# gau-nernst/llama-x

Measured on AMD Instinct MI355X. Metric: train tokens/sec Llama-3.1-8B seq4096 at 1/2/4/8 MI355X; p50 step ms, higher is better.
Workload: dtype bf16; 1 GPU; Llama-3.1-8B text-only LoRA r=16 bf16, seq=4096, 1 sequence per GPU, causal mask, base+LM head frozen (BASELINE.json configs[1]); random-init weights at 8B dimensions; seq_len=4096, parallelism=dp1, launch=hipGraph replay (fwd+bwd+AdamW), lm_head_rows=labelled only

## Files before the change

### llama-x_amd/csrc/attn_bwd.hip

```cpp
#include "attn.h"
#include "attn_dropout.h"

typedef __attribute__((ext_vector_type(8))) short s16x8_t;

__device__ __forceinline__ int dual_swz(int row) { return ((row & 3) << 2) | ((row >> 2) & 3); }
__device__ __forceinline__ uint32_t dual_swz(uint32_t row) { return ((row & 3) << 2) | ((row >> 2) & 3); }

__device__ __forceinline__ bf16x8_t tr_frag(const char* img, int row0, int db, int lane) {
  const int hh = lane >> 5, tq = (lane & 15) >> 2, tp = lane & 3, tsub = (lane >> 4) & 1;
  const int chunk = 4 * db + 2 * tsub + (tp >> 1);
  const int rlo = row0 + 4 * hh + tq, rhi = rlo + 8;
  s16x4_t lo = __builtin_amdgcn_ds_read_tr16_b64_v4i16((lds_s16x4*)(img + rlo * 256 + ((chunk ^ dual_swz(rlo)) << 4) + ((tp & 1) << 3)));
  s16x4_t hi = __builtin_amdgcn_ds_read_tr16_b64_v4i16((lds_s16x4*)(img + rhi * 256 + ((chunk ^ dual_swz(rhi)) << 4) + ((tp & 1) << 3)));
  s16x8_t v = {lo[0], lo[1], lo[2], lo[3], hi[0], hi[1], hi[2], hi[3]};
  return __builtin_bit_cast(bf16x8_t, v);
}

__device__ __forceinline__ bf16x8_t row_frag(const char* img, int row, int ks, int hh) {
  return *reinterpret_cast<const bf16x8_t*>(img + row * 256 + (((2 * ks + hh) ^ dual_swz(row)) << 4));
}

template <int N>
__device__ __forceinline__ void lds_tr_wait(s16x4_t& a, s16x4_t& b, s16x4_t (&c)[4], s16x4_t (&d)[4]) {
  asm volatile("s_waitcnt lgkmcnt(%10)"
               : "+v"(a), "+v"(b), "+v"(c[0]), "+v"(c[1]), "+v"(c[2]), "+v"(c[3]), "+v"(d[0]), "+v"(d[1]), "+v"(d[2]), "+v"(d[3])
               : "n"(N));
  __builtin_amdgcn_sched_barrier(0);
}
__device__ __forceinline__ uint32_t xor_imm(uint32_t a, int c) {
  if (c == 0) return a;
  uint32_t r;
  asm volatile("v_xor_b32 %0, %1, %2" : "=v"(r) : "n"(c), "v"(a));
  return r;
}

struct AttnBwdArgs {
  const bf16_t* q; const bf16_t* k; const bf16_t* v; const bf16_t* o; const bf16_t* d_o;
  const float* lse; float* delta; float* nlse;
  const float* rope;
  unsigned long long* stamps;
  bf16_t* dq; bf16_t* dk; bf16_t* dv;
  bf16_t* ds; int Sp;
  int64_t q_sb, q_ss, k_sb, k_ss, v_sb, v_ss, o_sb, o_ss, do_sb, do_ss;
  int64_t dq_sb, dq_ss, dk_sb, dk_ss, dv_sb, dv_ss;
  const int* doc_ids; const int* prefix_len; const uint8_t* flags;
  int B, S, H, KVH;
  float scale, scale_log2;
  const uint8_t* mask; int64_t m_sb, m_sq;
  const int64_t* rng; uint32_t drop_thr; float drop_c; int stream_id;
};

enum { BWD_CAUSAL = 0, BWD_RULE = 1, BWD_MASK = 2 };

__device__ __forceinline__ uint32_t mask_nibble(uint32_t w) {
  const uint32_t nz = (((w & 0x7f7f7f7fu) + 0x7f7f7f7fu) | w) & 0x80808080u;
  return ((nz >> 7) * 0x01020408u) >> 24;
}

#define DQ_STAGE_BYTES (2 * TILE_BYTES)
#define DQ_LDS_BYTES (2 * DQ_STAGE_BYTES)

template <int MODE, bool DROPOUT = false>
__global__ __launch_bounds__(256, 2) void attn_bwd_dq_kernel(const AttnBwdArgs a) {
  static_assert(!(DROPOUT && MODE == BWD_MASK), "dropout exists in the causal and the rule mode");
  constexpr bool GENERAL = MODE == BWD_RULE;
  constexpr bool FLAGS = MODE != BWD_CAUSAL;
  constexpr bool MASK = MODE == BWD_MASK;
  extern __shared__ __attribute__((aligned(256))) char smem[];
  const int tid = threadIdx.x, lane = tid & 63;
  const int wave = __builtin_amdgcn_readfirstlane(tid >> 6);
  const int nqb = (a.S + BQ - 1) / BQ, nkt = (a.S + BKV - 1) / BKV;
  const int qb = nqb - 1 - blockIdx.y;
  const int h = blockIdx.x, b = blockIdx.z;
  const int kvh = h / (a.H / a.KVH);
  const int r = lane & 31, hh = lane >> 5;
  const int qi = qb * BQ + wave * 32 + r;
  const int qrow = min(qi, a.S - 1);

  const uint8_t* fl = FLAGS ? a.flags + ((int64_t)b * nqb + qb) * nkt : nullptr;
  const int kt_end = FLAGS ? nkt : min(nkt, (qb * BQ + BQ + BKV - 1) / BKV);
  uint32_t fpack = 0;
  int fchunk = -1;
  auto tile_class = [&](int t) -> int {
    if constexpr (FLAGS) {
      if ((t >> 6) != fchunk) {
        fchunk = t >> 6;
        fpack = fl[min(fchunk * 64 + lane, nkt - 1)];
      }
      return __builtin_amdgcn_readlane((int)fpack, t & 63);
    } else {
      return (t * BKV + BKV - 1 <= qb * BQ) ? 2 : 1;
    }
  };
  auto next_tile = [&](int t) {
    while (t < kt_end && tile_class(t) == 0) ++t;
    return t;
  };

  const int srow_in = lane >> 4, sslot = lane & 15;
  const bf16_t* kbase = a.k + (int64_t)b * a.k_sb + kvh * HD;
  const bf16_t* vbase = a.v + (int64_t)b * a.v_sb + kvh * HD;
  uint32_t koff[4], voff[4];
#pragma unroll
  for (int i = 0; i < 4; ++i) {
    const int row = i * 16 + wave * 4 + srow_in;
    koff[i] = (uint32_t)(((int64_t)row * a.k_ss + (sslot ^ dual_swz(row)) * 8) * 2);
    voff[i] = (uint32_t)(((int64_t)row * a.v_ss + (sslot ^ (row & 15)) * 8) * 2);
  }
  auto stage = [&](int buf, int t) {
    char* sK = smem + buf * DQ_STAGE_BYTES;
    char* sV = sK + TILE_BYTES;
    if (t * BKV + BKV <= a.S) {
      const char* kt = (const char*)(kbase + (int64_t)t * BKV * a.k_ss);
      const char* vt = (const char*)(vbase + (int64_t)t * BKV * a.v_ss);
      if constexpr (DROPOUT) {
        uint32_t l0;
        asm volatile("v_mbcnt_lo_u32_b32 %0, -1, 0\n\tv_mbcnt_hi_u32_b32 %0, -1, %0" : "=v"(l0));
        const int slot = (int)(l0 & 15);
#pragma unroll
        for (int i = 0; i < 4; ++i) {
          const int row = i * 16 + wave * 4 + (int)(l0 >> 4);
          const uint32_t ko = (uint32_t)(((int64_t)row * a.k_ss + (slot ^ dual_swz(row)) * 8) * 2);
          const uint32_t vo = (uint32_t)(((int64_t)row * a.v_ss + (slot ^ (row & 15)) * 8) * 2);
          __builtin_amdgcn_global_load_lds((gbl_void*)(kt + ko), (lds_void*)(sK + (i * 16 + wave * 4) * 256), 16, 0, 0);
          __builtin_amdgcn_global_load_lds((gbl_void*)(vt + vo), (lds_void*)(sV + (i * 16 + wave * 4) * 256), 16, 0, 0);
        }
      } else {
#pragma unroll
      for (int i = 0; i < 4; ++i) {
        __builtin_amdgcn_global_load_lds((gbl_void*)(kt + koff[i]), (lds_void*)(sK + (i * 16 + wave * 4) * 256), 16, 0, 0);
        __builtin_amdgcn_global_load_lds((gbl_void*)(vt + voff[i]), (lds_void*)(sV + (i * 16 + wave * 4) * 256), 16, 0, 0);
      }
      }
    } else {
#pragma unroll
      for (int i = 0; i < 4; ++i) {
        const int row = i * 16 + wave * 4 + srow_in;
        const int key = min(t * BKV + row, a.S - 1);
        const int kc = sslot ^ dual_swz(row);
        const int vc = sslot ^ (row & 15);
        __builtin_amdgcn_global_load_lds((gbl_void*)(kbase + (int64_t)key * a.k_ss + kc * 8), (lds_void*)(sK + (i * 16 + wave * 4) * 256), 16, 0, 0);
        __builtin_amdgcn_global_load_lds((gbl_void*)(vbase + (int64_t)key * a.v_ss + vc * 8), (lds_void*)(sV + (i * 16 + wave * 4) * 256), 16, 0, 0);
      }
    }
  };

  const uint32_t sbase = (uint32_t)(uintptr_t)(__attribute__((address_space(3))) char*)smem;
  uint32_t aK0;
  {
    const int tq2 = (lane & 15) >> 2, tp = lane & 3, tsub = (lane >> 4) & 1;
    const int rlo = 4 * hh + tq2;
    aK0 = (uint32_t)(rlo * 256 + (((2 * tsub + (tp >> 1)) ^ dual_swz(rlo)) << 4) + ((tp & 1) << 3));
  }
  f32x16_t dq[4];
#pragma unroll
  for (int i = 0; i < 4; ++i)
#pragma unroll
    for (int e = 0; e < 16; ++e) dq[i][e] = 0.f;
  const int* docrow = (GENERAL && a.doc_ids) ? a.doc_ids + (int64_t)b * a.S : nullptr;
  const int my_doc = docrow ? docrow[qrow] : 0;
  const int my_prefix = (GENERAL && a.prefix_len) ? a.prefix_len[b] : 0;
  uint32_t mwn[MASK ? 8 : 1];
  auto mask_request = [&](int t_) {
    if constexpr (MASK) {
      uint32_t l0;
      asm volatile("v_mbcnt_lo_u32_b32 %0, -1, 0\n\tv_mbcnt_hi_u32_b32 %0, -1, %0" : "=v"(l0));
      const int hh = (int)(l0 >> 5);
      const uint8_t* mrow = a.mask + (int64_t)b * a.m_sb + (int64_t)min(qb * BQ + wave * 32 + (int)(l0 & 31), a.S - 1) * a.m_sq;
      if (t_ * BKV + BKV <= a.S) {
        const uint8_t* p = mrow + t_ * BKV + 4 * hh;
#pragma unroll
        for (int g = 0; g < 8; ++g) __builtin_memcpy(&mwn[g], p + (g >> 2) * 32 + 8 * (g & 3), 4);
      } else {
#pragma unroll
        for (int g = 0; g < 8; ++g) {
          const int g0 = t_ * BKV + (g >> 2) * 32 + 8 * (g & 3) + 4 * hh;
          __builtin_memcpy(&mwn[g], mrow + min(g0, a.S - 4), 4);
        }
      }
    }
  };
  auto mask_bits = [&](int t_) -> uint32_t {
    uint32_t bits = 0;
    if constexpr (MASK) {
      const bool ragged = t_ * BKV + BKV > a.S;
#pragma unroll
      for (int g = 0; g < 8; ++g) {
        uint32_t w = mwn[g];
        if (ragged) {
          const int g0 = t_ * BKV + (g >> 2) * 32 + 8 * (g & 3) + 4 * hh;
          const int sh = g0 - min(g0, a.S - 4);
          w = sh >= 4 ? 0u : w >> (8 * sh);
        }
        bits |= mask_nibble(w) << (4 * g);
      }
    }
    return bits;
  };

  int t = next_tile(0);
  if constexpr (MASK) {
#pragma unroll
    for (int g = 0; g < 8; ++g) mwn[g] = 0;
    if (t < kt_end && tile_class(t) == 1) mask_request(t);
  }
  if (t < kt_end) stage(0, t);
  bf16x8_t qf[8], dof[8], ovf[8];
  const float my_lse = a.lse[((int64_t)b * a.H + h) * a.S + qrow];
  {
    const bf16_t* qp = a.q + (int64_t)b * a.q_sb + (int64_t)qrow * a.q_ss + h * HD + 8 * hh;
    const bf16_t* dp = a.d_o + (int64_t)b * a.do_sb + (int64_t)qrow * a.do_ss + h * HD + 8 * hh;
    const bf16_t* op = a.o + (int64_t)b * a.o_sb + (int64_t)qrow * a.o_ss + h * HD + 8 * hh;
#pragma unroll
    for (int ks = 0; ks < 8; ++ks) {
      ovf[ks] = *reinterpret_cast<const bf16x8_t*>(op + 16 * ks);
      dof[ks] = *reinterpret_cast<const bf16x8_t*>(dp + 16 * ks);
      qf[ks] = *reinterpret_cast<const bf16x8_t*>(qp + 16 * ks);
    }
    __builtin_amdgcn_sched_barrier(0);
  }
  const float lse_safe = (my_lse == -INFINITY) ? 0.f : my_lse;
  float my_delta = 0.f;
  {
#pragma unroll
    for (int ks = 0; ks < 8; ++ks) {
#pragma unroll
      for (int j = 0; j < 8; ++j) my_delta += (float)ovf[ks][j] * (float)dof[ks][j];
    }
    my_delta += __shfl_xor(my_delta, 32, 64);
    if (hh == 0 && qi < a.S) {
      a.delta[((int64_t)b * a.H + h) * a.S + qi] = my_delta;
      a.nlse[((int64_t)b * a.H + h) * a.S + qi] = -lse_safe;
    }
  }

  asm volatile("s_waitcnt vmcnt(0)" ::: "memory");
  __syncthreads();
  int cur = 0;
  int docv = (GENERAL && docrow && t < kt_end) ? docrow[min(t * BKV + lane, a.S - 1)] : 0, docv_next = 0;
  AttnDropKey dkey = {0u, 0u};
  if constexpr (DROPOUT) dkey = attn_dropout_key(a.rng[0], a.rng[1], a.stream_id, b, h);
  while (t < kt_end) {
    int cls_m = 0;
    uint32_t mbits = 0;
    if constexpr (MASK) {
      cls_m = tile_class(t);
      if (cls_m == 1) mbits = mask_bits(t);
    }
    const int tn = next_tile(t + 1);
    if (tn < kt_end) stage(cur ^ 1, tn);
    if (GENERAL && docrow && tn < kt_end) docv_next = docrow[min(tn * BKV + lane, a.S - 1)];
    if constexpr (MASK) {
      if (tn < kt_end && tile_class(tn) == 1) mask_request(tn);
    }
    const char* sK = smem + cur * DQ_STAGE_BYTES;
    const char* sV = sK + TILE_BYTES;
    const int cls = MASK ? cls_m : tile_class(t);
#pragma unroll
    for (int kb = 0; kb < 2; ++kb) {
      f32x16_t st, dp;
      const f32x16_t zero = {0.f, 0.f, 0.f, 0.f, 0.f, 0.f, 0.f, 0.f, 0.f, 0.f, 0.f, 0.f, 0.f, 0.f, 0.f, 0.f};
      const int row = kb * 32 + r;
#pragma unroll
      for (int ks = 0; ks < 8; ++ks) {
        bf16x8_t kf = row_frag(sK, row, ks, hh);
        st = __builtin_amdgcn_mfma_f32_32x32x16_bf16(kf, qf[ks], ks == 0 ? zero : st, 0, 0, 0);
      }
      if (cls != 2) {
#pragma unroll
        for (int e = 0; e < 16; ++e) {
          if constexpr (MASK) {
            st[e] = ((mbits >> (kb * 16 + e)) & 1u) ? st[e] : -INFINITY;
          } else {
          const int kk = t * BKV + kb * 32 + (e & 3) + 8 * (e >> 2) + 4 * hh;
          bool ok = (kk < a.S) && (kk <= qi || kk < my_prefix);
          if constexpr (GENERAL) {
            const int kd = docrow ? __builtin_amdgcn_ds_bpermute((kk - t * BKV) << 2, docv) : my_doc;
            ok = ok && (kd == my_doc);
          }
          st[e] = ok ? st[e] : -INFINITY;
          }
        }
      }
#pragma unroll
      for (int e = 0; e < 16; ++e) st[e] = __builtin_amdgcn_exp2f(__builtin_fmaf(st[e], a.scale_log2, -lse_safe));
#pragma unroll
      for (int ks = 0; ks < 8; ++ks) {
        bf16x8_t vf = *reinterpret_cast<const bf16x8_t*>(sV + row * 256 + (((2 * ks + hh) ^ (row & 15)) << 4));
        dp = __builtin_amdgcn_mfma_f32_32x32x16_bf16(vf, dof[ks], ks == 0 ? zero : dp, 0, 0, 0);
      }
#pragma unroll
      for (int e = 0; e < 16; ++e) {
        float dpe = dp[e];
        if constexpr (DROPOUT) {
          const int kk = t * BKV + kb * 32 + (e & 3) + 8 * (e >> 2) + 4 * hh;
          dpe = attn_drop_keep(attn_drop_row(dkey, qi), attn_drop_col(dkey, kk), a.drop_thr) ? dpe * a.drop_c : 0.f;
        }
        st[e] = st[e] * (dpe - my_delta);
      }
      {
        const uint32_t kb_ = sbase + cur * DQ_STAGE_BYTES + kb * 8192 + aK0;
        s16x4_t Kl[4], Kh[4];
#pragma unroll
        for (int s = 0; s < 2; ++s) {
#pragma unroll
          for (int db = 0; db < 4; ++db) {
            if (s == 0) { lds_tr_read<0>(Kl[db], xor_imm(kb_, db << 6)); lds_tr_read<2048>(Kh[db], xor_imm(kb_, (db << 6) | 0x20)); }
            else { lds_tr_read<4096>(Kl[db], xor_imm(kb_, db << 6)); lds_tr_read<4096 + 2048>(Kh[db], xor_imm(kb_, (db << 6) | 0x20)); }
          }
          bf16x8_t dsb;
#pragma unroll
          for (int j = 0; j < 8; ++j) dsb[j] = (__bf16)st[8 * s + j];
          lds_tr_wait8<0>(Kl, Kh);
#pragma unroll
          for (int db = 0; db < 4; ++db) dq[db] = __builtin_amdgcn_mfma_f32_32x32x16_bf16(frag_of(Kl[db], Kh[db]), dsb, dq[db], 0, 0, 0);
          __builtin_amdgcn_sched_barrier(0);
        }
      }
    }
    asm volatile("s_waitcnt vmcnt(0)" ::: "memory");
    __syncthreads();
    cur ^= 1;
    t = tn;
    docv = docv_next;
  }

  if (qi < a.S) {
    bf16_t* op = a.dq + (int64_t)b * a.dq_sb + (int64_t)qi * a.dq_ss + h * HD;
    const bool wide = ((((uintptr_t)a.dq) | (uintptr_t)(a.dq_ss * 2) | (uintptr_t)(a.dq_sb * 2)) & 15) == 0;
#pragma unroll
    for (int db = 0; db < 4; ++db)
#pragma unroll
      for (int j2 = 0; j2 < 2; ++j2) {
        u32x2_t pp[2];
#pragma unroll
        for (int gg = 0; gg < 2; ++gg) {
          const int g4 = 2 * j2 + gg;
          u32x2_t pk;
          pk[0] = pack_bf2(dq[db][4 * g4 + 0] * a.scale, dq[db][4 * g4 + 1] * a.scale);
          pk[1] = pack_bf2(dq[db][4 * g4 + 2] * a.scale, dq[db][4 * g4 + 3] * a.scale);
          if (a.rope) {
            const f32x4_t t = *reinterpret_cast<const f32x4_t*>(a.rope + ((int64_t)qi * 64 + ((32 * db + 8 * g4 + 4 * hh) >> 1)) * 2);
            const float c0 = t[0], s0 = t[1] * -1.f, c1 = t[2], s1 = t[3] * -1.f;
            const float x0 = bflo(pk[0]), x1 = bfhi(pk[0]), y0 = bflo(pk[1]), y1 = bfhi(pk[1]);
            pk[0] = pack_bf2(x0 * c0 - x1 * s0, x1 * c0 + x0 * s0);
            pk[1] = pack_bf2(y0 * c1 - y1 * s1, y1 * c1 + y0 * s1);
          }
          pp[gg] = pk;
        }
        if (wide) {
          const auto r0 = __builtin_amdgcn_permlane32_swap(pp[0][0], pp[1][0], false, false);
          const auto r1 = __builtin_amdgcn_permlane32_swap(pp[0][1], pp[1][1], false, false);
          *reinterpret_cast<u32x4_t*>(op + 32 * db + 16 * j2 + 8 * hh) = u32x4_t{r0[0], r1[0], r0[1], r1[1]};
        } else {
          *reinterpret_cast<u32x2_t*>(op + 32 * db + 16 * j2 + 4 * hh) = pp[0];
          *reinterpret_cast<u32x2_t*>(op + 32 * db + 16 * j2 + 8 + 4 * hh) = pp[1];
        }
      }
  }
}

#define DKV_QT 64
#define DKV2_KEYS 128

typedef __attribute__((address_space(3))) char lds_char;
typedef __attribute__((address_space(3))) bf16x8_t lds_bf16x8;
typedef __attribute__((address_space(3))) f32x4_t lds_f32x4;
#define DKV3_LDS_BYTES (0x10000 + 1024)

template <int MODE, bool STAMP = false, bool DS = false, bool DROPOUT = false>
__global__ __launch_bounds__(256, 2) void attn_bwd_dkv3_kernel(const AttnBwdArgs a, float* __restrict__ part) {
  static_assert(!(DROPOUT && (MODE == BWD_MASK || STAMP || DS)), "dropout exists on the default route, in the causal and the rule mode");
  constexpr bool GENERAL = MODE == BWD_RULE;
  constexpr bool FLAGS = MODE != BWD_CAUSAL;
  constexpr bool MASK = MODE == BWD_MASK;
  static_assert(!(MASK && (STAMP || DS)), "the dense-mask mode exists on the default route only");
  extern __shared__ __attribute__((aligned(256))) char smem[];
  const int tid = threadIdx.x, lane = tid & 63;
  const int wave = __builtin_amdgcn_readfirstlane(tid >> 6);
  const int nqb = (a.S + BQ - 1) / BQ, nkt = (a.S + BKV - 1) / BKV;
  const int nqt = (a.S + DKV_QT - 1) / DKV_QT;
  const int G = a.H / a.KVH;
  int id = blockIdx.x;
  const int per_kb = a.B * a.KVH * G;
  const int kblk = id / per_kb;
  id -= kblk * per_kb;
  const int b = id / (a.KVH * G);
  id -= b * (a.KVH * G);
  const int kvh = id / G, g = id % G;
  const int h = kvh * G + g;
  const int my_kt = 2 * kblk + (wave >> 1);

  bf16x8_t kf[8], vf[8];
  const int* docrow = (GENERAL && a.doc_ids) ? a.doc_ids + (int64_t)b * a.S : nullptr;
  int key_doc = 0;
  {
    const int krow = min(kblk * DKV2_KEYS + wave * 32 + (lane & 31), a.S - 1);
    const bf16_t* kp = a.k + (int64_t)b * a.k_sb + (int64_t)krow * a.k_ss + kvh * HD + 8 * (lane >> 5);
    const bf16_t* vp = a.v + (int64_t)b * a.v_sb + (int64_t)krow * a.v_ss + kvh * HD + 8 * (lane >> 5);
#pragma unroll
    for (int ks = 0; ks < 8; ++ks) {
      kf[ks] = *reinterpret_cast<const bf16x8_t*>(kp + 16 * ks);
      vf[ks] = *reinterpret_cast<const bf16x8_t*>(vp + 16 * ks);
    }
    if (docrow) key_doc = docrow[krow];
  }
  const int my_prefix = (GENERAL && a.prefix_len) ? a.prefix_len[b] : 0;

  const int qt_first = FLAGS ? 0 : (kblk * DKV2_KEYS) / DKV_QT;
  uint32_t fpack = 0;
  int fchunk = -1;
  auto block_class = [&](int qt, int kt) -> int {
    if (kt >= nkt) return 0;
    if constexpr (FLAGS) {
      const int qb128 = qt >> 1;
      if ((qb128 >> 6) != fchunk) {
        fchunk = qb128 >> 6;
        uint32_t ln;
        asm volatile("v_mbcnt_lo_u32_b32 %0, -1, 0\n\tv_mbcnt_hi_u32_b32 %0, -1, %0" : "=v"(ln));
        const uint8_t* fr = a.flags + ((int64_t)b * nqb + min(fchunk * 64 + (int)ln, nqb - 1)) * nkt;
        fpack = (uint32_t)fr[2 * kblk] | ((2 * kblk + 1 < nkt ? (uint32_t)fr[2 * kblk + 1] : 0u) << 8);
      }
      const uint32_t w = (uint32_t)__builtin_amdgcn_readlane((int)fpack, qb128 & 63);
      return (int)((w >> (8 * (kt - 2 * kblk))) & 0xff);
    }
    const int q_lo = qt * DKV_QT, q_hi = q_lo + DKV_QT - 1, k_lo = kt * BKV, k_hi = k_lo + BKV - 1;
    if (k_lo > q_hi) return 0;
    return (k_hi <= q_lo) ? 2 : 1;
  };
  auto next_qt = [&](int qt) {
    while (qt < nqt && !(qt >= qt_first && (block_class(qt, 2 * kblk) != 0 || block_class(qt, 2 * kblk + 1) != 0))) ++qt;
    return qt;
  };

  const uint32_t sbase = (uint32_t)(uintptr_t)(lds_char*)smem;

  const char* qbase = (const char*)(a.q + (int64_t)b * a.q_sb + h * HD);
  const char* dbase = (const char*)(a.d_o + (int64_t)b * a.do_sb + h * HD);
  const float* lbase = (wave == 0 ? a.nlse : a.delta) + ((int64_t)b * a.H + h) * a.S;
  auto stage = [&](int buf, int qt) {
    uint32_t ln;
    asm volatile("v_mbcnt_lo_u32_b32 %0, -1, 0\n\tv_mbcnt_hi_u32_b32 %0, -1, %0" : "=v"(ln));
    const uint32_t srow = wave * 4 + (ln >> 4);
    const uint32_t sc = (ln & 15) ^ dual_swz(srow);
    lds_char* sQ = (lds_char*)smem + buf * 0x8000 + wave * 1024;
    if (qt * DKV_QT + DKV_QT <= a.S) {
      const uint32_t q_lane = (srow * (uint32_t)a.q_ss + sc * 8) * 2, d_lane = (srow * (uint32_t)a.do_ss + sc * 8) * 2;
#pragma unroll
      for (int i = 0; i < 4; ++i) {
        const char* qu = qbase + (int64_t)(qt * DKV_QT + i * 16) * a.q_ss * 2;
        const char* du = dbase + (int64_t)(qt * DKV_QT + i * 16) * a.do_ss * 2;
        __builtin_amdgcn_global_load_lds((gbl_void*)(qu + q_lane), (lds_void*)(sQ + i * 4096), 16, 0, 0);
        __builtin_amdgcn_global_load_lds((gbl_void*)(du + d_lane), (lds_void*)(sQ + 0x4000 + i * 4096), 16, 0, 0);
      }
    } else {
#pragma unroll
      for (int i = 0; i < 4; ++i) {
        const int qr = min(qt * DKV_QT + i * 16 + (int)srow, a.S - 1);
        __builtin_amdgcn_global_load_lds((gbl_void*)(qbase + ((int64_t)qr * a.q_ss + sc * 8) * 2), (lds_void*)(sQ + i * 4096), 16, 0, 0);
        __builtin_amdgcn_global_load_lds((gbl_void*)(dbase + ((int64_t)qr * a.do_ss + sc * 8) * 2), (lds_void*)(sQ + 0x4000 + i * 4096), 16, 0, 0);
      }
    }
    if (wave < 2) {
      const float* src = lbase + min(qt * DKV_QT + (int)ln, a.S - 1);
      __builtin_amdgcn_global_load_lds((gbl_void*)src, (lds_void*)((lds_char*)smem + 0x10000 + buf * 512 + wave * 256), 4, 0, 0);
    }
  };

  f32x16_t dk[4], dv[4];
#pragma unroll
  for (int i = 0; i < 4; ++i)
#pragma unroll
    for (int e = 0; e < 16; ++e) { dk[i][e] = 0.f; dv[i][e] = 0.f; }

  uint32_t mwn[MASK ? 8 : 1];
  auto mask_request = [&](int qt_) {
    if constexpr (MASK) {
      uint32_t l0;
      asm volatile("v_mbcnt_lo_u32_b32 %0, -1, 0\n\tv_mbcnt_hi_u32_b32 %0, -1, %0" : "=v"(l0));
      const uint8_t* mr = a.mask + (int64_t)b * a.m_sb + (int64_t)min(qt_ * DKV_QT + (int)l0, a.S - 1) * a.m_sq;
      const int key0 = kblk * DKV2_KEYS + wave * 32;
      if (key0 + 32 <= a.S) {
#pragma unroll
        for (int g = 0; g < 8; ++g) __builtin_memcpy(&mwn[g], mr + key0 + 4 * g, 4);
      } else {
#pragma unroll
        for (int g = 0; g < 8; ++g) __builtin_memcpy(&mwn[g], mr + min(key0 + 4 * g, a.S - 4), 4);
      }
    }
  };
  auto mask_bits = [&]() -> uint32_t {
    uint32_t bits = 0;
    if constexpr (MASK) {
#pragma unroll
      for (int g = 0; g < 8; ++g) asm volatile("" : "+v"(mwn[g]));
      const bool ragged = kblk * DKV2_KEYS + wave * 32 + 32 > a.S;
#pragma unroll
      for (int g = 0; g < 8; ++g) {
        uint32_t w = mwn[g];
        if (ragged) {
          const int g0 = kblk * DKV2_KEYS + wave * 32 + 4 * g;
          const int sh = g0 - min(g0, a.S - 4);
          w = sh >= 4 ? 0u : w >> (8 * sh);
        }
        bits |= mask_nibble(w) << (4 * g);
      }
    }
    return bits;
  };

  auto mask_wanted = [&](int qt_) -> bool {
    const int c = block_class(qt_, my_kt);
    return c == 1 || (c == 2 && qt_ * DKV_QT + DKV_QT > a.S);
  };
  int qt = next_qt(0);
  if constexpr (MASK) {
#pragma unroll
    for (int g = 0; g < 8; ++g) mwn[g] = 0;
    if (qt < nqt && mask_wanted(qt)) mask_request(qt);
  }
  int qdoc = 0, qdoc_next = 0;
  if (GENERAL && docrow && qt < nqt) {
    uint32_t l0;
    asm volatile("v_mbcnt_lo_u32_b32 %0, -1, 0\n\tv_mbcnt_hi_u32_b32 %0, -1, %0" : "=v"(l0));
    qdoc = docrow[min(qt * DKV_QT + (int)l0, a.S - 1)];
  }
  if (qt < nqt) stage(0, qt);
  asm volatile("s_waitcnt vmcnt(0)" ::: "memory");
  __syncthreads();
  int cur = 0;
  AttnDropKey dkey = {0u, 0u};
  if constexpr (DROPOUT) dkey = attn_dropout_key(a.rng[0], a.rng[1], a.stream_id, b, h);
  int nst = 0;
  auto stamp = [&]() {
    if constexpr (STAMP) {
      if (blockIdx.x == 0 && wave == 0 && nst < 1024) {
        unsigned long long tt;
        asm volatile("s_memtime %0\n\ts_waitcnt lgkmcnt(0)" : "=s"(tt) :: "memory");
        if (threadIdx.x == 0) a.stamps[nst] = tt;
        ++nst;
      }
    }
  };
  while (qt < nqt) {
    stamp();
    const int qtn = next_qt(qt + 1);
    const bool have_next = qtn < nqt;
    uint32_t ln;
    asm volatile("v_mbcnt_lo_u32_b32 %0, -1, 0\n\tv_mbcnt_hi_u32_b32 %0, -1, %0" : "=v"(ln));
    const uint32_t lr_ = ln & 31, lh_ = ln >> 5;
    const uint32_t Lr = sbase + cur * 0x8000 + lr_ * 256 + ((lh_ ^ dual_swz(lr_)) << 4);
    const uint32_t tq = (ln & 15) >> 2, tp = ln & 3, tsub = (ln >> 4) & 1, trow = 4 * lh_ + tq;
    const uint32_t Tl = sbase + cur * 0x8000 + trow * 256 + (((2 * tsub + (tp >> 1)) ^ dual_swz(trow)) << 4) + ((tp & 1) << 3);
    const uint32_t Th = sbase + cur * 0x8000 + (trow + 8) * 256 + (((2 * tsub + (tp >> 1)) ^ dual_swz(trow + 8)) << 4) + ((tp & 1) << 3);
    const uint32_t Ls = sbase + 0x10000 + cur * 512 + lh_ * 16;
    const int hh = (int)lh_;
    const int key = kblk * DKV2_KEYS + wave * 32 + (int)lr_;
    int cls = block_class(qt, my_kt);
    if (cls == 2 && (qt * DKV_QT + DKV_QT > a.S)) cls = 1;
    uint32_t rowbits = 0;
    if constexpr (MASK) {
      if (cls == 1) rowbits = mask_bits();
      __builtin_amdgcn_sched_barrier(0);
    }
    if (have_next) stage(cur ^ 1, qtn);
    if (GENERAL && docrow && have_next) qdoc_next = docrow[min(qtn * DKV_QT + (int)ln, a.S - 1)];
    stamp();
    if (cls != 0) {
      auto rowf = [&](int qb32, int img, int ks) -> bf16x8_t {
        return *(lds_bf16x8*)((lds_char*)(uintptr_t)xor_imm(Lr, ks << 5) + qb32 * 8192 + img * 0x4000);
      };
      auto trf = [&](int qb32, int img, int step, s16x4_t& tl, s16x4_t& th) {
        const int s2 = step >> 2, db = step & 3;
        lds_tr_read_rt(tl, xor_imm(Tl, db << 6), (qb32 * 32 + s2 * 16) * 256 + img * 0x4000);
        lds_tr_read_rt(th, xor_imm(Th, db << 6), (qb32 * 32 + s2 * 16) * 256 + img * 0x4000);
      };
#pragma unroll
      for (int qb32 = 0; qb32 < 2; ++qb32) {
        f32x16_t st, dp;
        const f32x16_t zero = {0.f, 0.f, 0.f, 0.f, 0.f, 0.f, 0.f, 0.f, 0.f, 0.f, 0.f, 0.f, 0.f, 0.f, 0.f, 0.f};
        bf16x8_t f3[3];
        f3[0] = rowf(qb32, 0, 0);
        f3[1] = rowf(qb32, 0, 1);
#pragma unroll
        for (int ks = 0; ks < 8; ++ks) {
          if (ks + 2 < 8) f3[(ks + 2) % 3] = rowf(qb32, 0, ks + 2);
          st = __builtin_amdgcn_mfma_f32_32x32x16_bf16(f3[ks % 3], kf[ks], ks == 0 ? zero : st, 0, 0, 0);
          __builtin_amdgcn_sched_barrier(0);
        }
        if (qb32 == 0) stamp();
        bf16x8_t g3[3];
        g3[0] = rowf(qb32, 1, 0);
        g3[1] = rowf(qb32, 1, 1);
        if (cls != 2) {
#pragma unroll
          for (int e = 0; e < 16; ++e) {
            const int qi = qt * DKV_QT + qb32 * 32 + 8 * (e >> 2) + 4 * hh + (e & 3);
            if constexpr (MASK) {
              const uint32_t rb = (uint32_t)__builtin_amdgcn_ds_bpermute((qi - qt * DKV_QT) << 2, (int)rowbits);
              st[e] = ((qi < a.S) && ((rb >> lr_) & 1u)) ? st[e] : -INFINITY;
            } else {
            bool ok = (qi < a.S) && (key < a.S) && (key <= qi || key < my_prefix);
            if constexpr (GENERAL) {
              const int qd = docrow ? __builtin_amdgcn_ds_bpermute((qi - qt * DKV_QT) << 2, qdoc) : key_doc;
              ok = ok && (qd == key_doc);
            }
            st[e] = ok ? st[e] : -INFINITY;
            }
          }
        }
#pragma unroll
        for (int g4 = 0; g4 < 4; ++g4) {
          const f32x4_t l4 = *(lds_f32x4*)((lds_char*)(uintptr_t)Ls + (qb32 * 32 + 8 * g4) * 4);
#pragma unroll
          for (int e2 = 0; e2 < 4; ++e2) st[4 * g4 + e2] = __builtin_amdgcn_exp2f(__builtin_fmaf(st[4 * g4 + e2], a.scale_log2, l4[e2]));
        }
        __builtin_amdgcn_sched_barrier(0);
        if (qb32 == 0) stamp();
#pragma unroll
        for (int ks = 0; ks < 8; ++ks) {
          if (ks + 2 < 8) g3[(ks + 2) % 3] = rowf(qb32, 1, ks + 2);
          dp = __builtin_amdgcn_mfma_f32_32x32x16_bf16(g3[ks % 3], vf[ks], ks == 0 ? zero : dp, 0, 0, 0);
          __builtin_amdgcn_sched_barrier(0);
        }
        if (qb32 == 0) stamp();
        s16x4_t tdl[2], tdh[2], tql[2], tqh[2];
        if constexpr (!DROPOUT) {
          trf(qb32, 1, 0, tdl[0], tdh[0]);
          trf(qb32, 0, 0, tql[0], tqh[0]);
        }
        bf16x8_t pb[2], dsb[2];
#pragma unroll
        for (int g4 = 0; g4 < 4; ++g4) {
          const f32x4_t d4 = *(lds_f32x4*)((lds_char*)(uintptr_t)Ls + 256 + (qb32 * 32 + 8 * g4) * 4);
#pragma unroll
          for (int e2 = 0; e2 < 4; ++e2) {
            const int e = 4 * g4 + e2;
            if constexpr (DROPOUT) {
              const int qi = qt * DKV_QT + qb32 * 32 + 8 * g4 + 4 * hh + e2;
              const bool keep = attn_drop_keep(attn_drop_row(dkey, qi), attn_drop_col(dkey, key), a.drop_thr);
              pb[e >> 3][e & 7] = (__bf16)(keep ? st[e] * a.drop_c : 0.f);
              dsb[e >> 3][e & 7] = (__bf16)(st[e] * ((keep ? dp[e] * a.drop_c : 0.f) - d4[e2]));
            } else {
            pb[e >> 3][e & 7] = (__bf16)st[e];
            dsb[e >> 3][e & 7] = (__bf16)(st[e] * (dp[e] - d4[e2]));
            }
          }
        }
        if constexpr (DS) {
          bf16_t* dtile = a.ds + ((int64_t)b * a.H + h) * a.Sp * a.Sp + (int64_t)(my_kt * (a.Sp >> 7) + (qt >> 1)) * (64 * 128);
#pragma unroll
          for (int s2 = 0; s2 < 2; ++s2) {
            const u32x4_t w = __builtin_bit_cast(u32x4_t, dsb[s2]);
            const auto r0 = __builtin_amdgcn_permlane32_swap(w[0], w[2], false, false);
            const auto r1 = __builtin_amdgcn_permlane32_swap(w[1], w[3], false, false);
            const int piece = ((((wave & 1) * 2 + (qt & 1)) * 2 + qb32) * 2 + s2) * 64;
            *reinterpret_cast<u32x4_t*>(dtile + (piece + (int)ln) * 8) = u32x4_t{r0[0], r1[0], r0[1], r1[1]};
          }
        }
        if constexpr (DROPOUT) {
          __builtin_amdgcn_sched_barrier(0);
          trf(qb32, 1, 0, tdl[0], tdh[0]);
          trf(qb32, 0, 0, tql[0], tqh[0]);
        }
        __builtin_amdgcn_sched_barrier(0);
        if (qb32 == 0) stamp();
#pragma unroll
        for (int step = 0; step < 8; ++step) {
          if (step + 1 < 8) {
            trf(qb32, 1, step + 1, tdl[(step + 1) & 1], tdh[(step + 1) & 1]);
            trf(qb32, 0, step + 1, tql[(step + 1) & 1], tqh[(step + 1) & 1]);
          }
          if (step + 1 < 8) lds_tr_wait4<4>(tdl[step & 1], tdh[step & 1], tql[step & 1], tqh[step & 1]);
          else lds_tr_wait4<0>(tdl[step & 1], tdh[step & 1], tql[step & 1], tqh[step & 1]);
          dv[step & 3] = __builtin_amdgcn_mfma_f32_32x32x16_bf16(frag_of(tdl[step & 1], tdh[step & 1]), pb[step >> 2], dv[step & 3], 0, 0, 0);
          dk[step & 3] = __builtin_amdgcn_mfma_f32_32x32x16_bf16(frag_of(tql[step & 1], tqh[step & 1]), dsb[step >> 2], dk[step & 3], 0, 0, 0);
          __builtin_amdgcn_sched_barrier(0);
        }
        if (qb32 == 0) stamp();
      }
    }
    if constexpr (MASK) {
#pragma unroll
      for (int g = 0; g < 8; ++g) mwn[g] = 0;
      if (have_next && mask_wanted(qtn)) mask_request(qtn);
    }
    stamp();
    asm volatile("s_waitcnt vmcnt(0)" ::: "memory");
    stamp();
    __syncthreads();
    stamp();
    cur ^= 1;
    qt = qtn;
    qdoc = qdoc_next;
  }

  const int64_t plane = (int64_t)a.B * a.S * a.KVH * HD;
  uint32_t le;
  asm volatile("v_mbcnt_lo_u32_b32 %0, -1, 0\n\tv_mbcnt_hi_u32_b32 %0, -1, %0" : "=v"(le));
  const int hh = (int)(le >> 5);
  const int key = kblk * DKV2_KEYS + wave * 32 + (int)(le & 31);
  if (key < a.S) {
    float* pk = part + (int64_t)(g * 2 + 0) * plane + (((int64_t)b * a.S + key) * a.KVH + kvh) * HD;
    float* pv = part + (int64_t)(g * 2 + 1) * plane + (((int64_t)b * a.S + key) * a.KVH + kvh) * HD;
#pragma unroll
    for (int db = 0; db < 4; ++db)
#pragma unroll
      for (int g4 = 0; g4 < 4; ++g4) {
        const int d = 32 * db + 8 * g4 + 4 * hh;
        *reinterpret_cast<f32x4_t*>(pk + d) = f32x4_t{dk[db][4 * g4], dk[db][4 * g4 + 1], dk[db][4 * g4 + 2], dk[db][4 * g4 + 3]};
        *reinterpret_cast<f32x4_t*>(pv + d) = f32x4_t{dv[db][4 * g4], dv[db][4 * g4 + 1], dv[db][4 * g4 + 2], dv[db][4 * g4 + 3]};
      }
  }
}

__global__ __launch_bounds__(256) void attn_bwd_delta_kernel(const AttnBwdArgs a) {
  const int64_t idx = (int64_t)blockIdx.x * 16 + (threadIdx.x >> 4);
  const int c = threadIdx.x & 15;
  const int64_t total = (int64_t)a.B * a.S * a.H;
  const int64_t i = idx < total ? idx : total - 1;
  const int h = (int)(i % a.H);
  const int64_t bq = i / a.H;
  const int q = (int)(bq % a.S), b = (int)(bq / a.S);
  const u32x4_t ov = *reinterpret_cast<const u32x4_t*>(a.o + (int64_t)b * a.o_sb + (int64_t)q * a.o_ss + h * HD + c * 8);
  const u32x4_t dv = *reinterpret_cast<const u32x4_t*>(a.d_o + (int64_t)b * a.do_sb + (int64_t)q * a.do_ss + h * HD + c * 8);
  float s = 0.f;
#pragma unroll
  for (int e = 0; e < 4; ++e) s += bflo(ov[e]) * bflo(dv[e]) + bfhi(ov[e]) * bfhi(dv[e]);
  s += __shfl_xor(s, 1, 64);
  s += __shfl_xor(s, 2, 64);
  s += __shfl_xor(s, 4, 64);
  s += __shfl_xor(s, 8, 64);
  if (c == 0 && idx < total) {
    const int64_t o = ((int64_t)b * a.H + h) * a.S + q;
    const float l = a.lse[o];
    a.delta[o] = s;
    a.nlse[o] = (l == -INFINITY) ? 0.f : -l;
  }
}

#define DQ2_BQ 256
#define DQ2_STAGE_BYTES (3 * TILE_BYTES)
#define DQ2_STAGES 3
#define DQ2_LDS_BYTES (DQ2_STAGES * DQ2_STAGE_BYTES)

template <bool GENERAL>
__global__ __launch_bounds__(512, 2) void attn_bwd_dq2_kernel(const AttnBwdArgs a) {
  extern __shared__ __attribute__((aligned(256))) char smem[];
  const int tid = threadIdx.x, lane = tid & 63;
  const int wave = __builtin_amdgcn_readfirstlane(tid >> 6);
  const int nqb = (a.S + BQ - 1) / BQ, nkt = (a.S + BKV - 1) / BKV;
  const int nqb2 = (a.S + DQ2_BQ - 1) / DQ2_BQ;
  const int qb2 = nqb2 - 1 - blockIdx.y;
  const int h = blockIdx.x, b = blockIdx.z;
  const int kvh = h / (a.H / a.KVH);
  const int r = lane & 31, hh = lane >> 5;
  const int qi = qb2 * DQ2_BQ + wave * 32 + r;
  const int my_qb = min(2 * qb2 + (wave >> 2), nqb - 1);

  const int kt_end = GENERAL ? nkt : min(nkt, (qb2 * DQ2_BQ + DQ2_BQ + BKV - 1) / BKV);
  unsigned long long fa0 = 0, fa1 = 0, fb0 = 0, fb1 = 0;
  if constexpr (GENERAL) {
    const uint8_t* fla = a.flags + ((int64_t)b * nqb + min(2 * qb2, nqb - 1)) * nkt;
    const uint8_t* flb = a.flags + ((int64_t)b * nqb + min(2 * qb2 + 1, nqb - 1)) * nkt;
    const bool has_b = 2 * qb2 + 1 < nqb;
    fa0 = __builtin_amdgcn_ballot_w64(lane < nkt && fla[min(lane, nkt - 1)] != 0);
    fa1 = __builtin_amdgcn_ballot_w64(64 + lane < nkt && fla[min(64 + lane, nkt - 1)] != 0);
    fb0 = __builtin_amdgcn_ballot_w64(has_b && lane < nkt && flb[min(lane, nkt - 1)] != 0);
    fb1 = __builtin_amdgcn_ballot_w64(has_b && 64 + lane < nkt && flb[min(64 + lane, nkt - 1)] != 0);
  }
  const unsigned long long fm0 = fa0 | fb0, fm1 = fa1 | fb1;
  auto next_tile = [&](int t) {
    if constexpr (GENERAL) {
      if (t < 64) {
        const unsigned long long m = fm0 >> t;
        if (m) return t + (int)__builtin_ctzll(m);
        t = 64;
      }
      if (t < 128) {
        const unsigned long long m = fm1 >> (t - 64);
        if (m) return t + (int)__builtin_ctzll(m);
      }
      return kt_end;
    }
    return t;
  };
  const unsigned long long my0 = (wave >> 2) ? fb0 : fa0, my1 = (wave >> 2) ? fb1 : fa1;
  const int my_last = 4 * qb2 + (wave >> 1);
  auto mine = [&](int t) -> bool {
    if constexpr (GENERAL) return t < 64 ? ((my0 >> t) & 1) != 0 : ((my1 >> (t - 64)) & 1) != 0;
    return t <= my_last;
  };

  const int srow_in = lane >> 4, sslot = lane & 15;
  const bf16_t* kbase = a.k + (int64_t)b * a.k_sb + kvh * HD;
  const bf16_t* dbase = a.ds + ((int64_t)b * a.H + h) * a.Sp * a.Sp + (int64_t)(2 * qb2) * (64 * 128);
  const int64_t dtile = (int64_t)(a.Sp >> 7) * (64 * 128);
  uint32_t koff[2];
#pragma unroll
  for (int i = 0; i < 2; ++i) {
    const int row = (i * 8 + wave) * 4 + srow_in;
    koff[i] = (uint32_t)(((int64_t)row * a.k_ss + (sslot ^ dual_swz(row)) * 8) * 2);
  }
  auto stage = [&](int buf, int t) {
    char* sK = smem + buf * DQ2_STAGE_BYTES;
    char* sD = sK + TILE_BYTES;
    const char* dt = (const char*)(dbase + t * dtile) + lane * 16;
#pragma unroll
    for (int i = 0; i < 4; ++i) __builtin_amdgcn_global_load_lds((gbl_void*)(dt + (i * 8 + wave) * 1024), (lds_void*)(sD + (i * 8 + wave) * 1024), 16, 0, 0);
    if (t * BKV + BKV <= a.S) {
      const char* kt = (const char*)(kbase + (int64_t)t * BKV * a.k_ss);
#pragma unroll
      for (int i = 0; i < 2; ++i) __builtin_amdgcn_global_load_lds((gbl_void*)(kt + koff[i]), (lds_void*)(sK + (i * 8 + wave) * 1024), 16, 0, 0);
    } else {
#pragma unroll
      for (int i = 0; i < 2; ++i) {
        const int row = (i * 8 + wave) * 4 + srow_in;
        const int key = min(t * BKV + row, a.S - 1);
        __builtin_amdgcn_global_load_lds((gbl_void*)(kbase + (int64_t)key * a.k_ss + (sslot ^ dual_swz(row)) * 8), (lds_void*)(sK + (i * 8 + wave) * 1024), 16, 0, 0);
      }
    }
  };

  const uint32_t sbase = (uint32_t)(uintptr_t)(lds_char*)smem;
  uint32_t aK_lo[4], aK_hi[4], aD;
  {
    const int tq2 = (lane & 15) >> 2, tp = lane & 3, tsub = (lane >> 4) & 1;
    const int rlo = 4 * hh + tq2, rhi = rlo + 8;
    auto off = [&](int row, int blk) { return (uint32_t)(row * 256 + (((4 * blk + 2 * tsub + (tp >> 1)) ^ dual_swz(row)) << 4) + ((tp & 1) << 3)); };
#pragma unroll
    for (int db = 0; db < 4; ++db) { aK_lo[db] = off(rlo, db); aK_hi[db] = off(rhi, db); }
    aD = (uint32_t)(TILE_BYTES + (wave >> 2) * TILE_BYTES + ((wave >> 1) & 1) * 4096 + (wave & 1) * 2048 + tsub * 1024 + (tp >> 1) * 512 + rlo * 16 + (tp & 1) * 8);
  }
  f32x16_t dq[4];
#pragma unroll
  for (int i = 0; i < 4; ++i)
#pragma unroll
    for (int e = 0; e < 16; ++e) dq[i][e] = 0.f;

  int tq[DQ2_STAGES];
  tq[0] = next_tile(0);
#pragma unroll
  for (int i = 1; i < DQ2_STAGES; ++i) tq[i] = tq[i - 1] < kt_end ? next_tile(tq[i - 1] + 1) : kt_end;
#pragma unroll
  for (int i = 0; i < DQ2_STAGES - 1; ++i)
    if (tq[i] < kt_end) stage(i, tq[i]);
  int cur = 0;
  while (tq[0] < kt_end) {
    if (tq[2] < kt_end) {
      stage((cur + 2) % DQ2_STAGES, tq[2]);
      asm volatile("s_waitcnt vmcnt(12)" ::: "memory");
    } else if (tq[1] < kt_end) {
      asm volatile("s_waitcnt vmcnt(6)" ::: "memory");
    } else {
      asm volatile("s_waitcnt vmcnt(0)" ::: "memory");
    }
    __builtin_amdgcn_s_barrier();
    asm volatile("" ::: "memory");
    if (mine(tq[0])) {
      const uint32_t so = sbase + cur * DQ2_STAGE_BYTES;
      s16x4_t Dl[2], Dh[2], Kl[2][4], Kh[2][4];
      auto reads = [&](auto set_tag, auto ks_tag) {
        constexpr int st = decltype(set_tag)::value, ks = decltype(ks_tag)::value, off = ks * 4096, doff_ = (ks >> 1) * 8192 + (ks & 1) * 256;
        lds_tr_read<doff_>(Dl[st], so + aD);
        lds_tr_read<doff_ + 128>(Dh[st], so + aD);
#pragma unroll
        for (int db = 0; db < 4; ++db) {
          lds_tr_read<off>(Kl[st][db], so + aK_lo[db]);
          lds_tr_read<off>(Kh[st][db], so + aK_hi[db]);
        }
      };
      auto mfmas = [&](auto set_tag) {
        constexpr int st = decltype(set_tag)::value;
        const bf16x8_t dsf = frag_of(Dl[st], Dh[st]);
#pragma unroll
        for (int db = 0; db < 4; ++db) dq[db] = __builtin_amdgcn_mfma_f32_32x32x16_bf16(frag_of(Kl[st][db], Kh[st][db]), dsf, dq[db], 0, 0, 0);
        __builtin_amdgcn_sched_barrier(0);
      };
// ... 222 lines not shown
```

Measured before the change: 32770 tokens/s.

## Replace XOR-swizzled LDS tiles with padded dual-piece layout in attention backward

```diff
diff --git a/llama-x_amd/csrc/attn_bwd.hip b/llama-x_amd/csrc/attn_bwd.hip
--- a/llama-x_amd/csrc/attn_bwd.hip
+++ b/llama-x_amd/csrc/attn_bwd.hip
@@ -16,8 +16,15 @@
   return __builtin_bit_cast(bf16x8_t, v);
 }
 
-__device__ __forceinline__ bf16x8_t row_frag(const char* img, int row, int ks, int hh) {
-  return *reinterpret_cast<const bf16x8_t*>(img + row * 256 + (((2 * ks + hh) ^ dual_swz(row)) << 4));
+#define DUAL_PIECE_BYTES 1040
+#define DUAL_IMG_BYTES (16 * DUAL_PIECE_BYTES)
+__device__ __forceinline__ constexpr uint32_t dual_pos(uint32_t slot) { return ((slot & 3) << 2) | (slot >> 2); }
+__device__ __forceinline__ constexpr uint32_t dual_off(uint32_t row, uint32_t slot) { return (row & 15) * DUAL_PIECE_BYTES + (row >> 4) * 256 + dual_pos(slot) * 16; }
+__device__ __forceinline__ uint32_t dual_dma_row(uint32_t lane) { return 16 * (lane >> 4); }
+__device__ __forceinline__ uint32_t dual_dma_slot(uint32_t lane) { return dual_pos(lane & 15); }
+__device__ __forceinline__ uint32_t dual_tr_base(uint32_t lane) {
+  const uint32_t hh = lane >> 5, tq = (lane & 15) >> 2, tp = lane & 3, tsub = (lane >> 4) & 1;
+  return dual_off(4 * hh + tq, 2 * tsub + (tp >> 1)) + ((tp & 1) << 3);
 }
 
 template <int N>
@@ -26,12 +33,6 @@
                : "+v"(a), "+v"(b), "+v"(c[0]), "+v"(c[1]), "+v"(c[2]), "+v"(c[3]), "+v"(d[0]), "+v"(d[1]), "+v"(d[2]), "+v"(d[3])
                : "n"(N));
   __builtin_amdgcn_sched_barrier(0);
-}
-__device__ __forceinline__ uint32_t xor_imm(uint32_t a, int c) {
-  if (c == 0) return a;
-  uint32_t r;
-  asm volatile("v_xor_b32 %0, %1, %2" : "=v"(r) : "n"(c), "v"(a));
-  return r;
 }
 
 struct AttnBwdArgs {
@@ -57,7 +58,7 @@
   return ((nz >> 7) * 0x01020408u) >> 24;
 }
 
-#define DQ_STAGE_BYTES (2 * TILE_BYTES)
+#define DQ_STAGE_BYTES (2 * DUAL_IMG_BYTES)
 #define DQ_LDS_BYTES (2 * DQ_STAGE_BYTES)
 
 template <int MODE, bool DROPOUT = false>
@@ -97,61 +98,55 @@
     return t;
   };
 
-  const int srow_in = lane >> 4, sslot = lane & 15;
+  const int srow_in = (int)dual_dma_row((uint32_t)lane) + wave, sslot = (int)dual_dma_slot((uint32_t)lane);
   const bf16_t* kbase = a.k + (int64_t)b * a.k_sb + kvh * HD;
   const bf16_t* vbase = a.v + (int64_t)b * a.v_sb + kvh * HD;
   uint32_t koff[4], voff[4];
 #pragma unroll
   for (int i = 0; i < 4; ++i) {
-    const int row = i * 16 + wave * 4 + srow_in;
-    koff[i] = (uint32_t)(((int64_t)row * a.k_ss + (sslot ^ dual_swz(row)) * 8) * 2);
-    voff[i] = (uint32_t)(((int64_t)row * a.v_ss + (sslot ^ (row & 15)) * 8) * 2);
+    const int row = 4 * i + srow_in;
+    koff[i] = (uint32_t)(((int64_t)row * a.k_ss + sslot * 8) * 2);
+    voff[i] = (uint32_t)(((int64_t)row * a.v_ss + sslot * 8) * 2);
   }
   auto stage = [&](int buf, int t) {
-    char* sK = smem + buf * DQ_STAGE_BYTES;
-    char* sV = sK + TILE_BYTES;
+    char* sK = smem + buf * DQ_STAGE_BYTES + wave * DUAL_PIECE_BYTES;
+    char* sV = sK + DUAL_IMG_BYTES;
     if (t * BKV + BKV <= a.S) {
       const char* kt = (const char*)(kbase + (int64_t)t * BKV * a.k_ss);
       const char* vt = (const char*)(vbase + (int64_t)t * BKV * a.v_ss);
       if constexpr (DROPOUT) {
         uint32_t l0;
         asm volatile("v_mbcnt_lo_u32_b32 %0, -1, 0\n\tv_mbcnt_hi_u32_b32 %0, -1, %0" : "=v"(l0));
-        const int slot = (int)(l0 & 15);
+        const int slot = (int)dual_dma_slot(l0);
 #pragma unroll
         for (int i = 0; i < 4; ++i) {
-          const int row = i * 16 + wave * 4 + (int)(l0 >> 4);
-          const uint32_t ko = (uint32_t)(((int64_t)row * a.k_ss + (slot ^ dual_swz(row)) * 8) * 2);
-          const uint32_t vo = (uint32_t)(((int64_t)row * a.v_ss + (slot ^ (row & 15)) * 8) * 2);
-          __builtin_amdgcn_global_load_lds((gbl_void*)(kt + ko), (lds_void*)(sK + (i * 16 + wave * 4) * 256), 16, 0, 0);
-          __builtin_amdgcn_global_load_lds((gbl_void*)(vt + vo), (lds_void*)(sV + (i * 16 + wave * 4) * 256), 16, 0, 0);
+          const int row = (int)((4 * i + wave) + dual_dma_row(l0));
+          const uint32_t ko = (uint32_t)(((int64_t)row * a.k_ss + slot * 8) * 2);
+          const uint32_t vo = (uint32_t)(((int64_t)row * a.v_ss + slot * 8) * 2);
+          __builtin_amdgcn_global_load_lds((gbl_void*)(kt + ko), (lds_void*)(sK + i * 4 * DUAL_PIECE_BYTES), 16, 0, 0);
+          __builtin_amdgcn_global_load_lds((gbl_void*)(vt + vo), (lds_void*)(sV + i * 4 * DUAL_PIECE_BYTES), 16, 0, 0);
         }
       } else {
 #pragma unroll
       for (int i = 0; i < 4; ++i) {
-        __builtin_amdgcn_global_load_lds((gbl_void*)(kt + koff[i]), (lds_void*)(sK + (i * 16 + wave * 4) * 256), 16, 0, 0);
-        __builtin_amdgcn_global_load_lds((gbl_void*)(vt + voff[i]), (lds_void*)(sV + (i * 16 + wave * 4) * 256), 16, 0, 0);
+        __builtin_amdgcn_global_load_lds((gbl_void*)(kt + koff[i]), (lds_void*)(sK + i * 4 * DUAL_PIECE_BYTES), 16, 0, 0);
+        __builtin_amdgcn_global_load_lds((gbl_void*)(vt + voff[i]), (lds_void*)(sV + i * 4 * DUAL_PIECE_BYTES), 16, 0, 0);
       }
       }
     } else {
 #pragma unroll
       for (int i = 0; i < 4; ++i) {
-        const int row = i * 16 + wave * 4 + srow_in;
+        const int row = 4 * i + srow_in;
         const int key = min(t * BKV + row, a.S - 1);
-        const int kc = sslot ^ dual_swz(row);
-        const int vc = sslot ^ (row & 15);
-        __builtin_amdgcn_global_load_lds((gbl_void*)(kbase + (int64_t)key * a.k_ss + kc * 8), (lds_void*)(sK + (i * 16 + wave * 4) * 256), 16, 0, 0);
-        __builtin_amdgcn_global_load_lds((gbl_void*)(vbase + (int64_t)key * a.v_ss + vc * 8), (lds_void*)(sV + (i * 16 + wave * 4) * 256), 16, 0, 0);
+        __builtin_amdgcn_global_load_lds((gbl_void*)(kbase + (int64_t)key * a.k_ss + sslot * 8), (lds_void*)(sK + i * 4 * DUAL_PIECE_BYTES), 16, 0, 0);
+        __builtin_amdgcn_global_load_lds((gbl_void*)(vbase + (int64_t)key * a.v_ss + sslot * 8), (lds_void*)(sV + i * 4 * DUAL_PIECE_BYTES), 16, 0, 0);
       }
     }
   };
 
   const uint32_t sbase = (uint32_t)(uintptr_t)(__attribute__((address_space(3))) char*)smem;
-  uint32_t aK0;
-  {
-    const int tq2 = (lane & 15) >> 2, tp = lane & 3, tsub = (lane >> 4) & 1;
-    const int rlo = 4 * hh + tq2;
-    aK0 = (uint32_t)(rlo * 256 + (((2 * tsub + (tp >> 1)) ^ dual_swz(rlo)) << 4) + ((tp & 1) << 3));
-  }
+  const uint32_t aR0 = dual_off((uint32_t)r, (uint32_t)hh);
+  const uint32_t aK0 = dual_tr_base((uint32_t)lane);
   f32x16_t dq[4];
 #pragma unroll
   for (int i = 0; i < 4; ++i)
@@ -253,17 +248,16 @@
     if constexpr (MASK) {
       if (tn < kt_end && tile_class(tn) == 1) mask_request(tn);
     }
-    const char* sK = smem + cur * DQ_STAGE_BYTES;
-    const char* sV = sK + TILE_BYTES;
+    const char* sK = smem + cur * DQ_STAGE_BYTES + aR0;
+    const char* sV = sK + DUAL_IMG_BYTES;
     const int cls = MASK ? cls_m : tile_class(t);
 #pragma unroll
     for (int kb = 0; kb < 2; ++kb) {
       f32x16_t st, dp;
       const f32x16_t zero = {0.f, 0.f, 0.f, 0.f, 0.f, 0.f, 0.f, 0.f, 0.f, 0.f, 0.f, 0.f, 0.f, 0.f, 0.f, 0.f};
-      const int row = kb * 32 + r;
 #pragma unroll
       for (int ks = 0; ks < 8; ++ks) {
-        bf16x8_t kf = row_frag(sK, row, ks, hh);
+        bf16x8_t kf = *reinterpret_cast<const bf16x8_t*>(sK + dual_off(32 * kb, 2 * ks));
         st = __builtin_amdgcn_mfma_f32_32x32x16_bf16(kf, qf[ks], ks == 0 ? zero : st, 0, 0, 0);
       }
       if (cls != 2) {
@@ -286,7 +280,7 @@
       for (int e = 0; e < 16; ++e) st[e] = __builtin_amdgcn_exp2f(__builtin_fmaf(st[e], a.scale_log2, -lse_safe));
 #pragma unroll
       for (int ks = 0; ks < 8; ++ks) {
-        bf16x8_t vf = *reinterpret_cast<const bf16x8_t*>(sV + row * 256 + (((2 * ks + hh) ^ (row & 15)) << 4));
+        bf16x8_t vf = *reinterpret_cast<const bf16x8_t*>(sV + dual_off(32 * kb, 2 * ks));
         dp = __builtin_amdgcn_mfma_f32_32x32x16_bf16(vf, dof[ks], ks == 0 ? zero : dp, 0, 0, 0);
       }
 #pragma unroll
@@ -299,14 +293,14 @@
         st[e] = st[e] * (dpe - my_delta);
       }
       {
-        const uint32_t kb_ = sbase + cur * DQ_STAGE_BYTES + kb * 8192 + aK0;
+        const uint32_t kb_ = sbase + cur * DQ_STAGE_BYTES + aK0;
         s16x4_t Kl[4], Kh[4];
 #pragma unroll
         for (int s = 0; s < 2; ++s) {
 #pragma unroll
           for (int db = 0; db < 4; ++db) {
-            if (s == 0) { lds_tr_read<0>(Kl[db], xor_imm(kb_, db << 6)); lds_tr_read<2048>(Kh[db], xor_imm(kb_, (db << 6) | 0x20)); }
-            else { lds_tr_read<4096>(Kl[db], xor_imm(kb_, db << 6)); lds_tr_read<4096 + 2048>(Kh[db], xor_imm(kb_, (db << 6) | 0x20)); }
+            lds_tr_read_rt(Kl[db], kb_, dual_off(32 * kb + 16 * s, 4 * db));
+            lds_tr_read_rt(Kh[db], kb_, dual_off(32 * kb + 16 * s + 8, 4 * db));
           }
           bf16x8_t dsb;
 #pragma unroll
@@ -366,7 +360,9 @@
 typedef __attribute__((address_space(3))) char lds_char;
 typedef __attribute__((address_space(3))) bf16x8_t lds_bf16x8;
 typedef __attribute__((address_space(3))) f32x4_t lds_f32x4;
-#define DKV3_LDS_BYTES (0x10000 + 1024)
+#define DKV3_STAGE_BYTES (2 * DUAL_IMG_BYTES)
+#define DKV3_STATS (2 * DKV3_STAGE_BYTES)
+#define DKV3_LDS_BYTES (DKV3_STATS + 1024)
 
 template <int MODE, bool STAMP = false, bool DS = false, bool DROPOUT = false>
 __global__ __launch_bounds__(256, 2) void attn_bwd_dkv3_kernel(const AttnBwdArgs a, float* __restrict__ part) {
@@ -441,29 +437,29 @@
   auto stage = [&](int buf, int qt) {
     uint32_t ln;
     asm volatile("v_mbcnt_lo_u32_b32 %0, -1, 0\n\tv_mbcnt_hi_u32_b32 %0, -1, %0" : "=v"(ln));
-    const uint32_t srow = wave * 4 + (ln >> 4);
-    const uint32_t sc = (ln & 15) ^ dual_swz(srow);
-    lds_char* sQ = (lds_char*)smem + buf * 0x8000 + wave * 1024;
+    const uint32_t srow = wave + dual_dma_row(ln);
+    const uint32_t sc = dual_dma_slot(ln);
+    lds_char* sQ = (lds_char*)smem + buf * DKV3_STAGE_BYTES + wave * DUAL_PIECE_BYTES;
     if (qt * DKV_QT + DKV_QT <= a.S) {
       const uint32_t q_lane = (srow * (uint32_t)a.q_ss + sc * 8) * 2, d_lane = (srow * (uint32_t)a.do_ss + sc * 8) * 2;
 #pragma unroll
       for (int i = 0; i < 4; ++i) {
-        const char* qu = qbase + (int64_t)(qt * DKV_QT + i * 16) * a.q_ss * 2;
-        const char* du = dbase + (int64_t)(qt * DKV_QT + i * 16) * a.do_ss * 2;
-        __builtin_amdgcn_global_load_lds((gbl_void*)(qu + q_lane), (lds_void*)(sQ + i * 4096), 16, 0, 0);
-        __builtin_amdgcn_global_load_lds((gbl_void*)(du + d_lane), (lds_void*)(sQ + 0x4000 + i * 4096), 16, 0, 0);
+        const char* qu = qbase + (int64_t)(qt * DKV_QT + 4 * i) * a.q_ss * 2;
+        const char* du = dbase + (int64_t)(qt * DKV_QT + 4 * i) * a.do_ss * 2;
+        __builtin_amdgcn_global_load_lds((gbl_void*)(qu + q_lane), (lds_void*)(sQ + i * 4 * DUAL_PIECE_BYTES), 16, 0, 0);
+        __builtin_amdgcn_global_load_lds((gbl_void*)(du + d_lane), (lds_void*)(sQ + DUAL_IMG_BYTES + i * 4 * DUAL_PIECE_BYTES), 16, 0, 0);
       }
     } else {
 #pragma unroll
       for (int i = 0; i < 4; ++i) {
-        const int qr = min(qt * DKV_QT + i * 16 + (int)srow, a.S - 1);
-        __builtin_amdgcn_global_load_lds((gbl_void*)(qbase + ((int64_t)qr * a.q_ss + sc * 8) * 2), (lds_void*)(sQ + i * 4096), 16, 0, 0);
-        __builtin_amdgcn_global_load_lds((gbl_void*)(dbase + ((int64_t)qr * a.do_ss + sc * 8) * 2), (lds_void*)(sQ + 0x4000 + i * 4096), 16, 0, 0);
+        const int qr = min(qt * DKV_QT + 4 * i + (int)srow, a.S - 1);
+        __builtin_amdgcn_global_load_lds((gbl_void*)(qbase + ((int64_t)qr * a.q_ss + sc * 8) * 2), (lds_void*)(sQ + i * 4 * DUAL_PIECE_BYTES), 16, 0, 0);
+        __builtin_amdgcn_global_load_lds((gbl_void*)(dbase + ((int64_t)qr * a.do_ss + sc * 8) * 2), (lds_void*)(sQ + DUAL_IMG_BYTES + i * 4 * DUAL_PIECE_BYTES), 16, 0, 0);
       }
     }
     if (wave < 2) {
       const float* src = lbase + min(qt * DKV_QT + (int)ln, a.S - 1);
-      __builtin_amdgcn_global_load_lds((gbl_void*)src, (lds_void*)((lds_char*)smem + 0x10000 + buf * 512 + wave * 256), 4, 0, 0);
+      __builtin_amdgcn_global_load_lds((gbl_void*)src, (lds_void*)((lds_char*)smem + DKV3_STATS + buf * 512 + wave * 256), 4, 0, 0);
     }
   };
 
@@ -549,11 +545,9 @@
     uint32_t ln;
     asm volatile("v_mbcnt_lo_u32_b32 %0, -1, 0\n\tv_mbcnt_hi_u32_b32 %0, -1, %0" : "=v"(ln));
     const uint32_t lr_ = ln & 31, lh_ = ln >> 5;
-    const uint32_t Lr = sbase + cur * 0x8000 + lr_ * 256 + ((lh_ ^ dual_swz(lr_)) << 4);
-    const uint32_t tq = (ln & 15) >> 2, tp = ln & 3, tsub = (ln >> 4) & 1, trow = 4 * lh_ + tq;
-    const uint32_t Tl = sbase + cur * 0x8000 + trow * 256 + (((2 * tsub + (tp >> 1)) ^ dual_swz(trow)) << 4) + ((tp & 1) << 3);
-    const uint32_t Th = sbase + cur * 0x8000 + (trow + 8) * 256 + (((2 * tsub + (tp >> 1)) ^ dual_swz(trow + 8)) << 4) + ((tp & 1) << 3);
-    const uint32_t Ls = sbase + 0x10000 + cur * 512 + lh_ * 16;
+    const uint32_t Lr = sbase + cur * DKV3_STAGE_BYTES + dual_off(lr_, lh_);
+    const uint32_t Tl = sbase + cur * DKV3_STAGE_BYTES + dual_tr_base(ln);
+    const uint32_t Ls = sbase + DKV3_STATS + cur * 512 + lh_ * 16;
     const int hh = (int)lh_;
     const int key = kblk * DKV2_KEYS + wave * 32 + (int)lr_;
     int cls = block_class(qt, my_kt);
@@ -568,12 +562,12 @@
     stamp();
     if (cls != 0) {
       auto rowf = [&](int qb32, int img, int ks) -> bf16x8_t {
-        return *(lds_bf16x8*)((lds_char*)(uintptr_t)xor_imm(Lr, ks << 5) + qb32 * 8192 + img * 0x4000);
+        return *(lds_bf16x8*)((lds_char*)(uintptr_t)Lr + dual_off(32 * qb32, 2 * ks) + img * DUAL_IMG_BYTES);
       };
       auto trf = [&](int qb32, int img, int step, s16x4_t& tl, s16x4_t& th) {
         const int s2 = step >> 2, db = step & 3;
-        lds_tr_read_rt(tl, xor_imm(Tl, db << 6), (qb32 * 32 + s2 * 16) * 256 + img * 0x4000);
-        lds_tr_read_rt(th, xor_imm(Th, db << 6), (qb32 * 32 + s2 * 16) * 256 + img * 0x4000);
+        lds_tr_read_rt(tl, Tl, dual_off(32 * qb32 + 16 * s2, 4 * db) + img * DUAL_IMG_BYTES);
+        lds_tr_read_rt(th, Tl, dual_off(32 * qb32 + 16 * s2 + 8, 4 * db) + img * DUAL_IMG_BYTES);
       };
 #pragma unroll
       for (int qb32 = 0; qb32 < 2; ++qb32) {
```

New measurement: 32890 tokens/s, median of 6. About the same (+0.4%).
